# kurhula/pyABC

Measured on AMD Instinct MI355X. Metric: accepted particles/sec/generation, higher is better.
Workload: dtype f32 (f16x3-limb MFMA, f32-grade)

## Files before the change

### include/abcgpu.h

```cpp
#ifndef ABCGPU_H
#define ABCGPU_H

#include <stddef.h>
#include <stdint.h>

#ifdef __cplusplus
extern "C" {
#endif

#define ABC_OK 0
#define ABC_ERR_INVALID (-1)
#define ABC_ERR_HIP (-2)
#define ABC_ERR_WORKSPACE (-3)
#define ABC_ERR_NOT_ENOUGH_PARTICLES (-4)
#define ABC_ERR_UNSUPPORTED (-5)
#define ABC_ERR_COMM (-6)

#define ABC_MAX_D 2048

#define ABC_PREC_F64 0
#define ABC_PREC_F32 1
#define ABC_PREC_X3 2

#define ABC_PRIOR_FLAT (-1)
// ... 76 lines not shown

int abc_mask_gave_up(double* dist, const int32_t* attempts, int64_t B,
                     int max_attempts, double value, void* stream);

size_t abc_compact_workspace(int64_t B);
int abc_accept_compact(const double* d, int64_t B, double eps, int64_t* idx,
                       int64_t* count, void* ws, size_t ws_bytes,
                       void* stream);
typedef struct abc_candidate_spec {
  int d;
  int S;
  const double* X;
  const double* cdf;
  const int32_t* guide;
  int64_t N;
  const double* L;
  int per_particle_L;
  const int32_t* prior_kind;
  const double* prior_params;
  int max_attempts;
  const int32_t* src;
  const double* a;
  const double* sigma;
  const double* x0;
  const double* wf;
  double p;
  uint64_t seed;
  uint32_t generation;
  const void* anc_table;
  const double* support_box;
} abc_candidate_spec;
int abc_prior_support_box(const int32_t* prior_kind, const double* prior_params, int d,
                          double* box, void* stream);
int64_t abc_ancestor_table_bytes(int64_t N, int d);
int abc_ancestor_table(const double* X, const double* cdf, int64_t N, int d,
                       void* table, size_t table_bytes, void* stream);
size_t abc_candidates_workspace(int64_t B);
int abc_candidates_round(const abc_candidate_spec* spec, int64_t idx0,
                         int64_t B, double eps, const double* eps_dev,
                         double eps_scale, int filter, int64_t cap,
                         int64_t* idx, int64_t* count, double* rec_x,
                         void* ws, size_t ws_bytes, void* stream);
int abc_round_keep(const int64_t* counts, int nranks, int rank, int64_t need, int64_t* keep,
                   void* stream);
int abc_candidates_regen(const abc_candidate_spec* spec, int64_t idx0,
                         const int64_t* idx, int64_t n, const int64_t* n_dev,
                         double* theta, double* prior_logpdf, int64_t* ancestor,
                         double* x, double* dist, void* stream);

size_t abc_candidates_propose_workspace(void);
int abc_candidates_propose(const abc_candidate_spec* spec, int64_t idx0, int64_t B,
                           double* theta, double* prior_logpdf, int64_t* ancestor,
                           int32_t* attempts, void* ws, size_t ws_bytes, void* stream);

int abc_pnorm_accept(const double* x, int64_t B, int S, const double* x0,
                     const double* wf, double p, double eps, const int32_t* attempts,
                     int max_attempts, int64_t cap, int64_t* idx, int64_t* count,
                     void* ws, size_t ws_bytes, void* stream);

#define ABC_AGG_MAX_TERMS 16
int abc_aggregate_distance(const double* x, int64_t B, int S, const double* x0,
                           const double* wf, const double* p, const double* c, int K,
                           double* d, double* terms, void* stream);
int abc_aggregate_accept(const double* x, int64_t B, int S, const double* x0,
                         const double* wf, const double* p, const double* c, int K,
                         double eps, const int32_t* attempts, int max_attempts, int64_t cap,
                         int64_t* idx, int64_t* count, void* ws, size_t ws_bytes,
// ... 120 lines not shown
```

### pyabc_amd/_native.py

```python
import ctypes as C
import os
import threading

_HERE = os.path.dirname(os.path.abspath(__file__))
LIB_PATH = os.environ.get("ABCGPU_LIB", os.path.join(_HERE, "libabcgpu.so"))

P = C.c_void_p
I64 = C.c_int64
I32 = C.c_int
D = C.c_double
U64 = C.c_uint64
U32 = C.c_uint32
SZ = C.c_size_t

SIGNATURES = {
    "abc_last_error": (C.c_char_p, []),
    "abc_version": (I32, []),
    "abc_profile_begin": (I32, []),
    "abc_profile_end": (I32, [P, P]),
    "abc_profile_channel": (I32, [I32, P, P]),
    "abc_weighted_moments_workspace": (SZ, [I64, I32]),
    "abc_weighted_moments": (I32, [P, P, I64, I32, P, P, SZ, P]),
    "abc_scan_workspace": (SZ, [I64]),
    "abc_inclusive_scan_f64": (I32, [P, P, I64, P, SZ, P]),
    "abc_normalize_weights_workspace": (SZ, [I64]),
    "abc_normalize_weights": (I32, [P, I64, P, P, SZ, P]),
    "abc_mvn_packed_bytes": (SZ, [I64, I32, I32]),
    "abc_mvn_x3_layout": (I32, [I32, P, P]),
    "abc_mvn_x3_max_exponent": (I32, []),
    "abc_mvn_pack_population": (I32, [P, P, I64, I32, P, P, I32, D, P, I32, P, P,
                                      P]),
    "abc_mvn_fit": (I32, [P, I32, D, I32, P, P, P, P, P, P, P]),
    "abc_mvn_logpdf_workspace": (SZ, [I64, I64, I32, I32]),
    "abc_mvn_logpdf": (I32, [P, I64, I32, P, P, P, I64, P, P, I32, I32, D, D,
                             P, P, P, SZ, P]),
    "abc_mvn_logpdf_direct": (I32, [P, I64, P, P, I64, I32, P, I32, P, I32,
                                    D, D, P, P]),
    "abc_cdf_guide": (I32, [P, I64, P, P]),
    "abc_ancestor_table_bytes": (I64, [I64, I32]),
    "abc_ancestor_table": (I32, [P, P, I64, I32, P, SZ, P]),
    "abc_propose": (I32, [P, P, P, I64, I32, P, P, P, U64, U32, I64, I64, I32,
                          P, P, P, P, P]),
    "abc_prior_logpdf": (I32, [P, I64, I32, P, P, P, P]),
    "abc_prior_uniforms": (I32, [P, P, I64, I32, U64, U32, I64, P]),
    "abc_simulate_linear_gaussian": (I32, [P, I64, I32, I32, P, P, P, U64,
                                           U32, I64, P, P]),
    "abc_pnorm": (I32, [P, I64, I32, P, P, D, P, P]),
    "abc_mask_gave_up": (I32, [P, P, I64, I32, D, P]),
    "abc_compact_workspace": (SZ, [I64]),
    "abc_accept_compact": (I32, [P, I64, D, P, P, P, SZ, P]),
    "abc_candidates_workspace": (SZ, [I64]),
    "abc_prior_support_box": (I32, [P, P, I32, P, P]),
    "abc_round_keep": (I32, [P, I32, I32, I64, P, P]),
    "abc_candidates_round": (I32, [P, I64, I64, D, P, D, I32, I64, P, P, P, P, SZ, P]),
    "abc_candidates_regen": (I32, [P, I64, P, I64, P, P, P, P, P, P, P]),
    "abc_pnorm_accept": (I32, [P, I64, I32, P, P, D, D, P, I32, I64, P, P, P, SZ, P]),
    "abc_aggregate_distance": (I32, [P, I64, I32, P, P, P, P, I32, P, P, P]),
    "abc_aggregate_accept": (I32, [P, I64, I32, P, P, P, P, I32, D, P, I32, I64, P, P, P,
                                   SZ, P]),
    "abc_column_span": (I32, [P, I64, I32, P, P, SZ, P]),
    "abc_whitened_norm": (I32, [P, I64, I32, P, P, P, P]),
    "abc_whitened_accept": (I32, [P, I64, I32, P, P, D, P, I32, I64, P, P, P, SZ, P]),
    "abc_column_gram": (I32, [P, I64, I32, P, P, P, SZ, P]),
    "abc_column_quantile": (I32, [P, I64, I32, D, P, P, SZ, P]),
    "abc_candidates_propose_workspace": (SZ, []),
    "abc_candidates_propose": (I32, [P, I64, I64, P, P, P, P, P, SZ, P]),
    "abc_gather_rows": (I32, [P, P, I64, I32, P, P]),
    "abc_gather_rows_batch": (I32, [I32, P, P, P, P, P, I64, P]),
    "abc_importance_weights": (I32, [P, P, P, I64, D, P, P]),
    "abc_sort_pairs_workspace": (SZ, [I64]),
    "abc_sort_pairs_f64": (I32, [P, P, I64, P, P, P, SZ, P]),
    "abc_weighted_quantile_workspace": (SZ, [I64]),
# ... 121 lines not shown
```

### pyabc_amd/csrc/abc_candidate.h

```cpp
#pragma once
#include "abc_common.h"

#pragma clang fp contract(off)

namespace abc {

constexpr double LOG_SQRT_2PI = 0.91893853320467274178;
constexpr uint32_t SLOTS_PER_ATTEMPT = 65536;
constexpr uint32_t SLOT_ANCESTOR = 0;
constexpr uint32_t SLOT_PERTURB = 1;
constexpr uint32_t SLOT_PRIOR = 32;
constexpr uint32_t SLOT_SIM = 0x40000000u;

__device__ __forceinline__ void normals4(uint64_t g, uint32_t slot, uint32_t gen,
                                         uint64_t seed, double n[4], int need = 4,
                                         const float* tab = BM_TAB) {
  u32x4 r = philox(g, slot, gen, seed);
  box_muller(r.x, r.y, n[0], n[1], tab);
  if (need > 2) box_muller(r.z, r.w, n[2], n[3], tab);
}

__device__ __forceinline__ void perturb_words(int p, const u32x4& anc, u32x4& r, uint64_t g,
                                              uint32_t s0, uint32_t gen, uint64_t seed,
                                              uint32_t& wa, uint32_t& wb) {
// ... 288 lines not shown
      const uint64_t new_lo = f == 0 ? lo : lo + step * (uint64_t)f;
      lo = new_lo;
      hi = new_hi;
    }
    return hi;
  };
  const uint64_t kc = dkey(c);
  uint64_t lo_key;
  if (prior_in_support1(kind, p, -INFINITY)) lo_key = dkey(-INFINITY);
  else lo_key = turn(dkey(-INFINITY), kc, true);
  uint64_t hi_key;
  if (prior_in_support1(kind, p, INFINITY)) hi_key = dkey(INFINITY);
  else hi_key = turn(kc, dkey(INFINITY), false) - 1;
  if (lane == 0) { lo_hi[0] = dval(lo_key); lo_hi[1] = dval(hi_key); }
}

struct ProposalArgs {
  const double* X;
  const double* cdf;
  const int32_t* guide;
  int64_t N;
  const double* L;
  const int32_t* kind;
  const double* params;
  int d;
  int max_attempts;
  uint64_t seed;
  uint32_t gen;
  const double* rec = nullptr;
  const int32_t* bguide = nullptr;
  int rs = 0;
  int64_t G = 0;
  const double* xmax = nullptr;
};

constexpr int ANC_HDR = 256;
__host__ __device__ inline int anc_rs(int d) { return (d + 1 + 15) / 16 * 16; }
__host__ __device__ inline int64_t anc_bins(int64_t N) {
  const int64_t g = 4 * N;
  return g < (int64_t)0x7FFFFFF0 ? g : (int64_t)0x7FFFFFF0;
}
__device__ __forceinline__ int64_t anc_bin(double x, double inv_step, int64_t G) {
  const double b = x * inv_step;
  return b >= (double)G ? G : (int64_t)b;
}

constexpr int PROP_MVN = 0, PROP_LOCAL = 1, PROP_PRIOR = 2;
using PropModes = std::integer_sequence<int, PROP_MVN, PROP_LOCAL, PROP_PRIOR>;
inline int proposal_mode(const double* X, bool per_particle_L) {
  return X == nullptr ? PROP_PRIOR : (per_particle_L ? PROP_LOCAL : PROP_MVN);
}

using CandDims = std::integer_sequence<int, 1, 2, 3, 4, 5, 6, 8, 10, 12, 16>;

template <class F>
void dispatch_candidate(int d, int mode, F&& f) {
  auto with_d = [&](auto D) { dispatch_int(PropModes{}, mode, [&](auto MODE) { f(D, MODE); }); };
  if (!dispatch_int(CandDims{}, d, with_d)) with_d(std::integral_constant<int, 0>{});
}

struct SimDistArgs {
  const int32_t* src;
  const double* a;
  const double* sigma;
  const double* x0;
  const double* wf;
  double p;
  int S;
};

constexpr int SIM_SMAX = 256;
constexpr int LT_DMAX = 16;
struct BlockConsts {
  float bmt[BM_TAB_SIZE];
  double LT[LT_DMAX * LT_DMAX];
  double box[2 * 64];
  double2 as[SIM_SMAX];
  double2 wx[SIM_SMAX];
// ... 2 lines not shown
  double inv_step;
  int lazy;
};

template <int D, int MODE, bool BOX_FROM_SRC = false>
__device__ __forceinline__ void stage_block_consts(BlockConsts& C, const ProposalArgs& A,
                                                   const SimDistArgs* M,
                                                   const double* box_src) {
  const int t = threadIdx.x, nt = blockDim.x;
  const int d = D > 0 ? D : A.d;
  for (int k = t; k < BM_TAB_SIZE; k += nt) C.bmt[k] = BM_TAB[k];
  if (MODE == PROP_MVN && D > 0 && D <= LT_DMAX)
    for (int e = t; e < d * d; e += nt) C.LT[(e % d) * d + e / d] = A.L[e];
  if (BOX_FROM_SRC) {
    for (int k = t; k < 2 * d; k += nt) C.box[k] = box_src[k];
  } else {
    for (int k = t >> 6; k < d; k += nt >> 6)
      support_bounds_wave(A.kind[k], A.params + 4 * k, C.box + 2 * k);
  }
  if (M)
    for (int k = t; k < M->S && k < SIM_SMAX; k += nt) {
      C.as[k] = make_double2(M->a[k], M->sigma[k]);
      C.wx[k] = make_double2(M->wf[k], M->x0[k]);
      C.src[k] = M->src[k];
    }
  if (t == 0) {
    const double total = (MODE != PROP_PRIOR) ? A.cdf[A.N - 1] : 0.0;
    C.total = total;
    C.inv_step = (MODE != PROP_PRIOR && A.rec) ? (double)A.G / total : 0.0;
  }
  __syncthreads();
}

template <int D, int MODE, bool TABLE = false>
__device__ __forceinline__ int propose_one(const ProposalArgs& A, const BlockConsts& C,
                                           uint64_t g, double* th, int64_t& j) {
  constexpr bool LT_LDS = MODE == PROP_MVN && D > 0 && D <= LT_DMAX;
  const int d = D > 0 ? D : A.d;
  j = -1;
  const double total = C.total;
  for (int att = 0; att < A.max_attempts; ++att) {
    const uint32_t s0 = (uint32_t)att * SLOTS_PER_ATTEMPT;
    int oz = 0;
    asm volatile("" : "+s"(oz));
    const double* LT = C.LT + oz;
    const double* box = C.box + oz;
    if (MODE == PROP_PRIOR) {
#pragma unroll
      for (int k = 0; k < (D > 0 ? D : d); ++k)
        th[k] = prior_draw1(A.kind[k], A.params + 4 * k, g,
                            s0 + SLOT_PRIOR + 512u * k, A.gen, A.seed);
    } else {
      const u32x4 ra = philox(g, s0 + SLOT_ANCESTOR, A.gen, A.seed);
      u32x4 r = ra;
      const double target = uniform53(ra.x, ra.y) * total;
      AncestorBracket br;
      if (TABLE) {
        const int64_t kt = anc_bin(target, C.inv_step, A.G);
        br = {A.bguide[kt], A.bguide[kt + 1]};
      } else {
        br = ancestor_bracket(A.guide, A.N, total, target);
      }
#pragma unroll
      for (int k = 0; k < (D > 0 ? D : d); ++k) th[k] = 0.0;
      const double* Lj = A.L;
      if (MODE == PROP_LOCAL) {
        j = TABLE ? table_finish(A.rec, A.rs, d, A.N, target, br)
                  : ancestor_finish(A.cdf, A.N, target, br);
        Lj = A.L + j * d * d;
      }
      auto pair = [&](int q) {
        uint32_t wa, wb;
        perturb_words(q >> 1, ra, r, g, s0, A.gen, A.seed, wa, wb);
        double n0, n1;
        box_muller(wa, wb, n0, n1, C.bmt);
        const bool two = q + 1 < d;
#pragma unroll
        for (int k = 0; k < (D > 0 ? D : d); ++k) {
          if (k >= q) {
            const double l0 = LT_LDS ? LT[q * d + k] : Lj[k * d + q];
            th[k] = fma(l0, n0, th[k]);
          }
          if (two && k >= q + 1) {
            const double l1 = LT_LDS ? LT[(q + 1) * d + k] : Lj[k * d + q + 1];
            th[k] = fma(l1, n1, th[k]);
          }
        }
      };
#pragma unroll 1
      for (int q = 0; q < d; q += 2) pair(q);
      if (MODE != PROP_LOCAL)
        j = TABLE ? table_finish(A.rec, A.rs, d, A.N, target, br)
                  : ancestor_finish(A.cdf, A.N, target, br);
      const double* Xj = TABLE ? A.rec + j * A.rs : A.X + j * d;
#pragma unroll
      for (int k = 0; k < (D > 0 ? D : d); ++k) th[k] = Xj[k] + th[k];
    }
    bool ok = true;
#pragma unroll
    for (int k = 0; k < (D > 0 ? D : d); ++k)
      ok = ok & (box[2 * k] <= th[k]) & (th[k] <= box[2 * k + 1]);
    if (ok) return att + 1;
  }
  return A.max_attempts + 1;
}

constexpr int LAZY_KT = 4;

template <int D, int MODE>
__device__ __forceinline__ bool lazy_filter_ok(const BlockConsts& C, const ProposalArgs& A,
                                               const SimDistArgs& M) {
  if constexpr (MODE != PROP_MVN || D <= LAZY_KT || D > LT_DMAX) {
    return false;
  } else {
    if (A.xmax == nullptr || M.S <= 4) return false;
    bool ok = true;
    for (int k = 0; k < 4; ++k) ok = ok && C.src[k] >= 0 && C.src[k] < LAZY_KT;
    const double xm = *A.xmax;
    for (int k = LAZY_KT; k < D; ++k) {
      double ls = 0.0;
      for (int q = 0; q <= k; ++q) ls += fabs(C.LT[q * D + k]);
      const double b = (xm + 7.6 * ls) * 1.000001 + 1e-300;
      ok = ok && (C.box[2 * k] <= -b) && (b <= C.box[2 * k + 1]);
    }
    return ok;
  }
}

__device__ __forceinline__ double pterm(double v, double p) {
#pragma clang fp contract(off)
  return (p == 1.0) ? v : (p == 2.0 ? v * v : pow(v, p));
}
template <int PK = 0>
__device__ __forceinline__ double pnorm_acc(double s, double v, double p) {
#pragma clang fp contract(off)
  if constexpr (PK == 2) return s + v * v;
  return isinf(p) ? fmax(s, v) : s + pterm(v, p);
}
template <int PK = 0>
__device__ __forceinline__ double pnorm_finish(double s, double p) {
#pragma clang fp contract(off)
  if constexpr (PK == 2) return sqrt(s);
  return isinf(p) ? s : ((p == 1.0) ? s : (p == 2.0 ? sqrt(s) : pow(s, 1.0 / p)));
}
__device__ __forceinline__ double pnorm_row(const double* xr, int S, const double* x0,
                                            const double* wf, double p) {
#pragma clang fp contract(off)
  double s = 0.0;
// ... 77 lines not shown
    double n2[2];
    box_muller((q & 2) ? r.z : r.x, (q & 2) ? r.w : r.y, n2[0], n2[1], C.bmt);
#pragma unroll
    for (int t = 0; t < 2; ++t) {
      const int k = q + t;
      if (k < q1) {
        const double2 as = C.as[k], wx = C.wx[k];
        const int sk = __builtin_amdgcn_readfirstlane(C.src[k]);
        const double xv = lg_stat(as.x, as.y, th[sk], n2[t]);
        if (x) x[k - xoff] = xv;
        s = pnorm_acc<PK>(s, fabs(wx.x * (xv - wx.y)), M.p);
      }
    }
  }
  return s;
}

template <int D, int PK = 0>
__device__ __forceinline__ double sim_pnorm(const SimDistArgs& M, const BlockConsts& C,
                                            const double* th, uint64_t g, uint32_t gen,
                                            uint64_t seed, int q0, int q1, double s, double* x,
                                            int xoff = 0) {
  if constexpr (D > 0) {
    return sim_pnorm_regs<D, PK>(M, C, *reinterpret_cast<const double(*)[D]>(th), g, gen, seed,
                                 q0, q1, s, x, xoff);
  } else {
    return sim_pnorm_range<PK>(M, C, th, 1, g, gen, seed, q0, q1, s, x, xoff);
  }
}

template <int D, int PK, int CG>
__device__ __forceinline__ void lazy_head_group(const ProposalArgs& A, const SimDistArgs& M,
                                                const BlockConsts& C, const uint64_t (&g)[CG],
                                                double eps, bool (&keep)[CG]) {
  constexpr int KT = LAZY_KT;
  static_assert(D > KT, "lazy_head_group: D > LAZY_KT");
  int oz = 0;
  asm volatile("" : "+s"(oz));
  const double* LT = C.LT + oz;
  const double* box = C.box + oz;
  double target[CG];
  int32_t glo[CG], ghi[CG];
  uint32_t az[CG], aw[CG];
#pragma unroll
  for (int c = 0; c < CG; ++c) {
    const u32x4 r = philox(g[c], SLOT_ANCESTOR, A.gen, A.seed);
    target[c] = uniform53(r.x, r.y) * C.total;
    az[c] = r.z;
    aw[c] = r.w;
    const int64_t kt = anc_bin(target[c], C.inv_step, A.G);
    glo[c] = A.bguide[kt];
    ghi[c] = A.bguide[kt + 1];
  }
  double th[CG][KT];
#pragma unroll
  for (int c = 0; c < CG; ++c) {
#pragma unroll
    for (int k = 0; k < KT; ++k) th[c][k] = 0.0;
    const u32x4 r = philox(g[c], SLOT_PERTURB, A.gen, A.seed);
#pragma unroll
    for (int q = 0; q < KT; q += 2) {
      double n0, n1;
      box_muller(q == 0 ? az[c] : r.x, q == 0 ? aw[c] : r.y, n0, n1, C.bmt);
#pragma unroll
      for (int k = 0; k < KT; ++k) {
        if (k >= q) th[c][k] = fma(LT[q * D + k], n0, th[c][k]);
        if (k >= q + 1) th[c][k] = fma(LT[(q + 1) * D + k], n1, th[c][k]);
      }
    }
  }
  const double* xh[CG];
#pragma unroll
  for (int c = 0; c < CG; ++c) {
    const int64_t j = table_finish(A.rec, A.rs, D, A.N, target[c],
                                   AncestorBracket{(int64_t)glo[c], (int64_t)ghi[c]});
    xh[c] = A.rec + j * A.rs;
  }
  double xv4[CG][KT];
#pragma unroll
  for (int c = 0; c < CG; ++c)
#pragma unroll
    for (int k = 0; k < KT; ++k) xv4[c][k] = xh[c][k];
  double e[CG][4];
#pragma unroll
  for (int c = 0; c < CG; ++c) {
    const u32x4 r = philox(g[c], SLOT_SIM, A.gen, A.seed);
    box_muller(r.x, r.y, e[c][0], e[c][1], C.bmt);
    box_muller(r.z, r.w, e[c][2], e[c][3], C.bmt);
  }
#pragma unroll
  for (int c = 0; c < CG; ++c) {
    bool ok = true;
#pragma unroll
    for (int k = 0; k < KT; ++k) {
      th[c][k] = xv4[c][k] + th[c][k];
      ok = ok & (box[2 * k] <= th[c][k]) & (th[c][k] <= box[2 * k + 1]);
    }
    double s = 0.0;
#pragma unroll
    for (int k = 0; k < 4; ++k) {
      const double2 as = C.as[k], wx = C.wx[k];
      const int sk = __builtin_amdgcn_readfirstlane(C.src[k]);
      const double xv = lg_stat(as.x, as.y, th[c][sk], e[c][k]);
      s = pnorm_acc<PK>(s, fabs(wx.x * (xv - wx.y)), M.p);
    }
    keep[c] = !ok || !(pnorm_finish<PK>(s, M.p) > eps);
  }
}

}
```

### pyabc_amd/csrc/abc_fused.hip

```cpp
#include "abc_candidate.h"
#include "abc_aggregate.h"
#include "abc_accept_words.h"

namespace abc {
namespace {

constexpr int FR_T = 256;
constexpr int FR_CPT = 8;
constexpr int FR_TILE = FR_T * FR_CPT;
constexpr int FR_WORDS = FR_TILE / 64;
constexpr int FR_CG = 2;

struct RoundArgs {
  ProposalArgs P;
  SimDistArgs M;
  const double* box;
  const double* eps_dev;
  double eps_scale;
};

template <int D, int MODE, int PK>
__device__ __forceinline__ double evaluate_full(const RoundArgs& A, const BlockConsts& C,
                                                uint64_t g,
                                                double* th, int64_t& j, int& att, double* x) {
  att = propose_one<D, MODE, true>(A.P, C, g, th, j);
  const double s = sim_pnorm<D, PK>(A.M, C, th, g, A.P.gen, A.P.seed, 0, A.M.S, 0.0, x);
  const double dist = pnorm_finish<PK>(s, A.M.p);
  return att <= A.P.max_attempts ? dist : NAN;
}

constexpr int XCH = 16;
template <int D, int MODE, int PK>
__device__ __forceinline__ double evaluate_staged(const RoundArgs& A, const BlockConsts& C,
                                                  uint64_t g, bool valid, double* th,
                                                  int64_t& j, int& att, double* out,
                                                  int nvalid, double (*stage)[XCH + 1]) {
  const int t = threadIdx.x;
  const int S = A.M.S;
  att = valid ? propose_one<D, MODE, true>(A.P, C, g, th, j) : A.P.max_attempts + 1;
  double s = 0.0;
  for (int k0 = 0; k0 < S; k0 += XCH) {
    const int k1 = k0 + XCH < S ? k0 + XCH : S;
    if (valid) s = sim_pnorm<D, PK>(A.M, C, th, g, A.P.gen, A.P.seed, k0, k1, s, stage[t], k0);
    __syncthreads();
    const int w = k1 - k0;
    for (int e = t; e < FR_T * w; e += FR_T) {
      const int r = e / w, c = e - r * w;
      if (r < nvalid) out[(int64_t)r * S + k0 + c] = stage[r][c];
    }
    __syncthreads();
  }
  const double dist = pnorm_finish<PK>(s, A.M.p);
  return att <= A.P.max_attempts ? dist : NAN;
}

__device__ __forceinline__ void flush_accept_words(const uint32_t* tbits, int nwords,
                                                   int64_t tile0, int64_t B, uint64_t* bits) {
  const int lane = threadIdx.x & 63, wave = threadIdx.x >> 6;
  if (wave == 0 && lane < nwords) {
    const uint64_t w = (uint64_t)tbits[2 * lane] | ((uint64_t)tbits[2 * lane + 1] << 32);
    const int64_t word = tile0 / 64 + lane;
    if (word * 64 < B) bits[word] = w;
  }
}

struct TileLds {
  uint32_t* tbits;
  uint16_t* queue;
  int& qn;
};
template <int D, int MODE, bool FILTER, int PK>
__device__ __forceinline__ void tile_body(const RoundArgs& A, const BlockConsts& C, double eps,
                                          int64_t idx0, int64_t B, int64_t tile0, int cpt,
                                          uint64_t* __restrict__ bits,
                                          double* __restrict__ rec_x, TileLds T) {
  constexpr int DM = D > 0 ? D : 64;
  const int tid = threadIdx.x;
  const int tn = cpt * FR_T;
  if (tid < tn / 32) T.tbits[tid] = 0u;
  if (tid == 0) T.qn = 0;
  __syncthreads();
  double th[DM];
  int64_t j;
  int att;
  if (FILTER) {
    bool lazy_done = false;
    if constexpr (MODE == PROP_MVN && D > LAZY_KT && D <= LT_DMAX) {
      if (C.lazy) {
#pragma unroll 1
        for (int it = 0; it < cpt; it += FR_CG) {
          uint64_t gs[FR_CG];
          bool keep[FR_CG];
#pragma unroll
          for (int c = 0; c < FR_CG; ++c) gs[c] = (uint64_t)(idx0 + tile0 + (it + c) * FR_T + tid);
          lazy_head_group<D, PK, FR_CG>(A.P, A.M, C, gs, eps, keep);
#pragma unroll
          for (int c = 0; c < FR_CG; ++c) {
            const int loc = (it + c) * FR_T + tid;
            if (keep[c] && tile0 + loc < B) {
              const int pos = atomicAdd(&T.qn, 1);
              T.queue[pos] = (uint16_t)loc;
            }
          }
        }
        lazy_done = true;
      }
    }
#pragma unroll 1
    for (int it = 0; it < (lazy_done ? 0 : cpt); ++it) {
      const int loc = it * FR_T + tid;
      const int64_t b = tile0 + loc;
      if (b < B) {
        const uint64_t g = (uint64_t)(idx0 + b);
        att = propose_one<D, MODE, true>(A.P, C, g, th, j);
        const double s = sim_pnorm<D, PK>(A.M, C, th, g, A.P.gen, A.P.seed, 0, 4, 0.0, nullptr);
        if (att <= A.P.max_attempts && !(pnorm_finish<PK>(s, A.M.p) > eps)) {
          const int pos = atomicAdd(&T.qn, 1);
          T.queue[pos] = (uint16_t)loc;
        }
      }
    }
    __syncthreads();
  }
  const int n = FILTER ? T.qn : tn;
#pragma unroll 1
  for (int i = tid; i < n; i += FR_T) {
    const int loc = FILTER ? (int)T.queue[i] : i;
    const int64_t b = tile0 + loc;
    if (b < B) {
      double* xr = rec_x ? rec_x + b * A.M.S : nullptr;
      const double dist = evaluate_full<D, MODE, PK>(A, C, (uint64_t)(idx0 + b), th, j, att,
                                                  xr);
      if (dist <= eps) atomicOr(&T.tbits[loc >> 5], 1u << (loc & 31));
    }
  }
  __syncthreads();
  flush_accept_words(T.tbits, tn / 64, tile0, B, bits);
}

constexpr int FR_CPT_TAIL = 2;
constexpr int FR_TILE_TAIL = FR_T * FR_CPT_TAIL;

struct TilePlan {
  int64_t nbig, ntiles;
  unsigned int grid;
};
__host__ __device__ inline void tile_span(int64_t t, int64_t nbig, int64_t& tile0, int& cpt) {
  if (t < nbig) { tile0 = t * FR_TILE; cpt = FR_CPT; }
  else { tile0 = nbig * FR_TILE + (t - nbig) * FR_TILE_TAIL; cpt = FR_CPT_TAIL; }
}

template <int D, int MODE, bool FILTER, int PK>
__device__ __forceinline__ void round_body(RoundArgs A, int64_t idx0, int64_t B,
                                           double eps_host, uint64_t* __restrict__ bits,
                                           unsigned int* __restrict__ ticket,
                                           int64_t nbig, int64_t ntiles,
                                           double* __restrict__ rec_x) {
  const double eps = A.eps_dev ? (*A.eps_dev) * A.eps_scale : eps_host;
  __shared__ BlockConsts C;
  __shared__ uint32_t tbits[FR_TILE / 32];
  __shared__ uint16_t queue[FR_TILE];
  __shared__ int qn;
  __shared__ int64_t s_tile;
  const TileLds T{tbits, queue, qn};
  stage_block_consts<D, MODE, true>(C, A.P, &A.M, A.box);
  if (FILTER) {
    if (threadIdx.x == 0) C.lazy = lazy_filter_ok<D, MODE>(C, A.P, A.M) ? 1 : 0;
  }
  const unsigned int limit = (unsigned int)(ntiles + gridDim.x - 1);
#pragma unroll 1
  for (;;) {
    if (threadIdx.x == 0) s_tile = (int64_t)atomicInc(ticket, limit);
    __syncthreads();
    const int64_t t = s_tile;
    if (t >= ntiles) break;
    int64_t tile0;
    int cpt;
    tile_span(t, nbig, tile0, cpt);
    tile_body<D, MODE, FILTER, PK>(A, C, eps, idx0, B, tile0, cpt, bits, rec_x, T);
    __syncthreads();
  }
}

template <int D, int MODE, int PK>
__device__ __forceinline__ void round_plain_body(RoundArgs A, int64_t idx0, int64_t B,
                                                 double eps_host, uint64_t* __restrict__ bits,
                                                 unsigned int* __restrict__ ticket,
                                                 int64_t nbig, int64_t ntiles,
                                                 double* __restrict__ rec_x) {
  const double eps = A.eps_dev ? (*A.eps_dev) * A.eps_scale : eps_host;
  constexpr int DM = D > 0 ? D : 64;
  __shared__ BlockConsts C;
  __shared__ uint32_t tbits[FR_TILE / 32];
  __shared__ int64_t s_tile;
  stage_block_consts<D, MODE, true>(C, A.P, &A.M, A.box);
  const int tid = threadIdx.x, lane = tid & 63, wave = tid >> 6;
  const unsigned int limit = (unsigned int)(ntiles + gridDim.x - 1);
// ... 383 lines not shown
  unsigned long long a = 0ull;
  for (int64_t e = (int64_t)blockIdx.x * 256 + threadIdx.x; e < n; e += (int64_t)gridDim.x * 256) {
    const unsigned long long b = (unsigned long long)__double_as_longlong(fabs(X[e]));
    a = b > a ? b : a;
  }
#pragma unroll
  for (int o = 32; o > 0; o >>= 1) {
    const unsigned long long b = __shfl_xor(a, o, 64);
    a = b > a ? b : a;
  }
  if ((threadIdx.x & 63) == 0) wm[threadIdx.x >> 6] = a;
  __syncthreads();
  if (threadIdx.x == 0) {
    unsigned long long m = 0ull;
    for (int w = 0; w < 4; ++w) m = wm[w] > m ? wm[w] : m;
    atomicMax(xmax_bits, m);
  }
}

__global__ __launch_bounds__(256) void anc_guide_kernel(const double* __restrict__ cdf,
                                                        int64_t N, int64_t G,
                                                        int32_t* __restrict__ guide) {
  const int64_t k = (int64_t)blockIdx.x * 256 + threadIdx.x;
  if (k > G + 1) return;
  const double inv_step = (double)G / cdf[N - 1];
  int64_t lo = 0, hi = N;
  while (lo < hi) {
    const int64_t mid = (lo + hi) >> 1;
    if (anc_bin(cdf[mid], inv_step, G) >= k) hi = mid; else lo = mid + 1;
  }
  guide[k] = (int32_t)lo;
}

struct AncTable { const double* rec; const int32_t* guide; int rs; int64_t G; const double* xmax; };
inline AncTable anc_table_view(const void* t, int64_t N, int d) {
  AncTable v;
  v.xmax = static_cast<const double*>(t);
  v.rs = anc_rs(d);
  v.G = anc_bins(N);
  v.rec = reinterpret_cast<const double*>(static_cast<const char*>(t) + ANC_HDR);
  v.guide = reinterpret_cast<const int32_t*>(v.rec + N * v.rs);
  return v;
}

RoundArgs round_args(const abc_candidate_spec* s, const double* box) {
  RoundArgs A;
  A.box = box;
  A.eps_dev = nullptr;
  A.eps_scale = 1.0;
  A.P = ProposalArgs{s->X, s->cdf, s->guide, s->N, s->L, s->prior_kind,
                     s->prior_params, s->d, s->max_attempts, s->seed, s->generation};
  if (s->X && s->anc_table) {
    const AncTable v = anc_table_view(s->anc_table, s->N, s->d);
    A.P.rec = v.rec;
    A.P.bguide = v.guide;
    A.P.rs = v.rs;
    A.P.G = v.G;
    A.P.xmax = v.xmax;
  }
  A.M = SimDistArgs{s->src, s->a, s->sigma, s->x0, s->wf, s->p, s->S};
  return A;
}

int check_spec(const abc_candidate_spec* s) {
  ABC_CHECK_ARG(s != nullptr, "candidates: null spec");
  ABC_CHECK_ARG(s->d >= 1 && s->d <= 64 && s->S >= 1, "candidates: bad d/S");
  if (s->S > SIM_SMAX)
    return set_error(ABC_ERR_UNSUPPORTED, "candidates: S > %d (use the staged kernels)",
                     SIM_SMAX);
  ABC_CHECK_ARG(s->max_attempts >= 1 && s->max_attempts < (1 << 15),
                "candidates: bad max_attempts");
  ABC_CHECK_ARG(s->prior_kind && s->prior_params && s->src && s->a && s->sigma && s->x0 &&
                s->wf, "candidates: null pointer");
  ABC_CHECK_ARG(s->X == nullptr || (s->cdf && s->L && s->N >= 1),
                "candidates: population needs cdf, L, N");
  ABC_CHECK_ARG(s->p >= 1.0, "candidates: p < 1");
  ABC_CHECK_ARG(s->X == nullptr || s->anc_table, "candidates: population needs anc_table");
  return ABC_OK;
}

template <class F>
void dispatch_spec(const abc_candidate_spec* spec, F&& f) {
  dispatch_candidate(spec->d, proposal_mode(spec->X, spec->per_particle_L != 0), f);
}

}
}

using namespace abc;

struct RoundWs {
  unsigned int* ticket; int64_t* rtot; double* box; uint64_t* bits;
  void carve(Carver& c, int64_t B) {
    ticket = c.take<unsigned int>(64);
    rtot = c.take<int64_t>(RG_MAX);
    box = c.take<double>(128);
    bits = c.take<uint64_t>((size_t)ceil_div(B > 0 ? B : 1, FR_TILE) * FR_WORDS);
  }
};

extern "C" size_t abc_candidates_workspace(int64_t B) { return measure<RoundWs>(B); }

bool abc::accept_words_carve(void* ws, size_t ws_bytes, int64_t B, AcceptWords& w) {
  Carver cv(ws, ws_bytes);
  RoundWs r;
  r.carve(cv, B);
  w.bits = r.bits;
  w.rtot = r.rtot;
  return cv.ok;
}
int abc::accept_words_compact(const AcceptWords& w, int64_t B, int64_t cap, int64_t* idx,
                              int64_t* count, hipStream_t s) {
  return compact_accept_bits(w.bits, w.rtot, B, cap, idx, count, s);
}

extern "C" int64_t abc_ancestor_table_bytes(int64_t N, int d) {
  if (N < 1 || d < 1) return 0;
  return ANC_HDR + N * anc_rs(d) * (int64_t)sizeof(double) +
         (anc_bins(N) + 2) * (int64_t)sizeof(int32_t);
}

extern "C" int abc_ancestor_table(const double* X, const double* cdf, int64_t N, int d,
                                  void* table, size_t table_bytes, void* stream) {
  ABC_CHECK_ARG(N >= 1 && N < (1ll << 31) && d >= 1 && d <= 64,
                "ancestor_table: bad N/d");
  ABC_CHECK_ARG(X && cdf && table, "ancestor_table: null pointer");
  ABC_CHECK_ARG(((uintptr_t)table & 127) == 0, "ancestor_table: table not 128-B aligned");
  if ((int64_t)table_bytes < abc_ancestor_table_bytes(N, d))
    return set_error(ABC_ERR_WORKSPACE, "ancestor_table: buffer too small");
  const AncTable v = anc_table_view(table, N, d);
  hipStream_t s = as_stream(stream);
  ABC_HIP(hipMemsetAsync(table, 0, ANC_HDR, s));
  hipLaunchKernelGGL(anc_records_kernel, dim3((unsigned)ceil_div(N * v.rs, 256)), dim3(256), 0,
                     s, X, cdf, N, d, v.rs, const_cast<double*>(v.rec));
  ABC_LAUNCHED();
  const int64_t nx = N * (int64_t)d;
  const int64_t xb = ceil_div(nx, 256) < XMAX_BLOCKS ? ceil_div(nx, 256) : XMAX_BLOCKS;
  hipLaunchKernelGGL(anc_xmax_kernel, dim3((unsigned)xb), dim3(256), 0, s, X, nx,
                     static_cast<unsigned long long*>(table));
  ABC_LAUNCHED();
  hipLaunchKernelGGL(anc_guide_kernel, dim3((unsigned)ceil_div(v.G + 2, 256)), dim3(256), 0, s,
                     cdf, N, v.G, const_cast<int32_t*>(v.guide));
  ABC_LAUNCHED();
  return ABC_OK;
}

extern "C" int abc_candidates_round(const abc_candidate_spec* spec, int64_t idx0,
                                    int64_t B, double eps, const double* eps_dev,
                                    double eps_scale, int filter, int64_t cap,
                                    int64_t* idx, int64_t* count, double* rec_x,
                                    void* ws, size_t ws_bytes, void* stream) {
  const int rc = check_spec(spec);
  if (rc != ABC_OK) return rc;
  ABC_CHECK_ARG(B >= 0 && cap >= 0 && count, "candidates_round: bad B/cap/count");
  ABC_CHECK_ARG(B < (1ll << 40), "candidates_round: B too large");
  ABC_CHECK_ARG(cap == 0 || idx, "candidates_round: null idx");
  RoundWs w;
  ABC_CARVE(w, "candidates_round", B);
  hipStream_t s = as_stream(stream);
  if (B == 0) {
    ABC_HIP(hipMemsetAsync(count, 0, sizeof(int64_t), s));
    return ABC_OK;
  }
  const double p = spec->p;
  const int filt = (filter && rec_x == nullptr && spec->S > 4 &&
                    (p == 1.0 || p == 2.0 || p == INFINITY)) ? 1 : 0;
  const int64_t nt = ceil_div(B, FR_TILE);
  ABC_CHECK_ARG(nt < (1ll << 31), "candidates_round: too many tiles");
  const double* box = spec->support_box;
  if (!box) {
    hipLaunchKernelGGL(support_box_kernel, dim3((unsigned)spec->d), dim3(64), 0, s,
                       spec->prior_kind, spec->prior_params, spec->d, w.box);
    ABC_LAUNCHED();
    box = w.box;
  }
  RoundArgs A = round_args(spec, box);
// ... 153 lines not shown
```

### pyabc_amd/sampler/batched.py

```python
import logging
import math

import numpy as np

from .. import gpu
from .._native import PRIOR_KINDS
from ..distance.distance import SumStatMatrix
from ..population import ColumnarParticles, Particle, Population
from ..parameters import Parameter
from ..random_variables import host_prior_draw, host_prior_logpdf
from . import distributed as dd
from .base import Sampler

logger = logging.getLogger("Sampler")


class ColumnarSample:

    def __init__(self, columns, recorded, recorded_keys, record_rejected, ok,
                 accepted_flags=None, records=None):
        self._cols = columns
        self._records = records
        self._recorded = recorded
        self._recorded_keys = recorded_keys
# ... 361 lines not shown
        self.nr_evaluations_ = int(n_eval)
        self.last_stats = dict(rounds=0, evaluations=int(n_eval),
                               accepted=int(sample.n_accepted), per_candidate=True)
        return sample

    def _fused_round(self, spec, seed, gen, dev):
        if not self.fused or getattr(spec, "stochastic", None) is not None \
                or spec.distance is None or len(spec.param_names) > self.FUSED_MAX_DIM:
            return None
        if spec.transition is None and getattr(spec, "host_prior", None):
            return None
        sim = (spec.model.fused_simulator(dev)
               if hasattr(spec.model, "fused_simulator") else None)
        fp = (spec.distance.fused_pnorm(spec.t, spec.sum_stat_keys, dev)
              if hasattr(spec.distance, "fused_pnorm") else None)
        if sim is None or fp is None or len(spec.sum_stat_keys) > self.FUSED_MAX_STATS:
            return None
        prop = {}
        if spec.transition is not None:
            arrays = getattr(spec.transition, "proposal_arrays", None)
            if arrays is None:
                return None
            prop = arrays()
        src, a, sigma = sim
        wf, pval = fp
        fr = gpu.CandidateRound(len(spec.param_names), len(spec.sum_stat_keys),
                                spec.prior_kind, spec.prior_params, src, a,
                                sigma, spec.x0vec, wf, pval, seed, gen,
                                self.max_attempts, **prop)
        fr.src_host = getattr(spec.model, "src", None)
        return fr

    LAZY_KT = 4

    def _lazy_capable(self, spec, fr):
        s = fr.spec
        kinds = getattr(spec, "prior_kind_host", None)
        src = getattr(fr, "src_host", None)
        return (s.X is not None and not s.per_particle_L and s.d > self.LAZY_KT
                and s.S >= max(5, self.filter_min_stats) and s.p in (1.0, 2.0, math.inf)
                and kinds is not None
                and all(k in (PRIOR_KINDS["norm"], PRIOR_KINDS["laplace"])
                        for k in kinds)
                and src is not None and all(0 <= int(v) < self.LAZY_KT for v in src[:4]))

    FIRST_ROUND_SPARE = 4_000_000

    def _fused_size(self, need, ws, rate, measured, S, record):
        if self.batch_size is not None:
            return int(self.batch_size)
        r = rate if rate else 0.5
        if measured:
            mult = 1.06
        else:
            r *= self._acc_trend if rate else 1.0
            mult = 1.0 + min(0.1, self.FIRST_ROUND_SPARE * ws * max(r, 1e-12) / max(need, 1))
        b = need / max(r, 1e-12) * mult / ws + 4096
        cap = self.max_fused_batch_size
        if record:
            cap = min(cap, max(self.record_budget_bytes // (8 * S), 4096))
        return int(min(max(b, 4096), cap))

    def _limit_to_max_eval(self, B, max_eval, n_eval, ws):
        if not self.check_max_eval or not np.isfinite(max_eval):
            return B
        left = int(math.ceil(max_eval)) - int(n_eval)
        return int(max(1, min(B, left // ws)))

    def _ledger(self, n, rank, ws, S):
        return _RoundLedger(n, rank, ws, S, self.max_nr_recorded,
                            self.record_device_budget_bytes)

    def _sample_fused(self, n, fr, spec, max_eval, record, dev, rank, ws):
        torch = gpu.torch
        S = len(spec.sum_stat_keys)
        rec_x = []
        arena, arena_off = None, 0
        kept, kept_off, kept_segs = None, 0, []
        row_bytes = (8 * fr.d, 8, 8, 8 * S, 8)
        led = self._ledger(n, rank, ws, S)
        rate, measured = self._acc_rate, False
        tot_B = tot_cnt = 0
        filtered = reruns = 0
        while led.need > 0:
            if self.check_max_eval and led.n_eval >= max_eval:
                break
            need = led.need
            B = self._limit_to_max_eval(self._fused_size(need, ws, rate, measured, S, record),
                                        max_eval, led.n_eval, ws)
            kk = min(need, B)
            lo, _ = dd.rank_range(led.base, B, rank)
            rx = None
            if record and led.rec_left > 0:
                if arena is None or arena_off + B > arena.shape[0]:
                    arena = torch.empty((int(B * 1.25) + 4096, S), dtype=gpu.F64, device=dev)
                    arena_off = 0
                rx = arena[arena_off:arena_off + B]
            filt = (rate is not None and rate < self.filter_below and rx is None
                    and self._lazy_capable(spec, fr))
            filtered += int(filt)
            thr = getattr(spec, "eps_device", None) if led.rounds == 0 else None
            if thr is not None:
                idx, cnt = fr.run(lo, B, 0.0, cap=need, filter=filt, rec_x=rx,
                                  eps_dev=thr[0], eps_scale=thr[1])
            else:
                idx, cnt = fr.run(lo, B, spec.eps, cap=need, filter=filt, rec_x=rx)
            if ws == 1:
                n_keep = cnt
                self._reader.queue(cnt, idx[kk - 1:kk])
            else:
                gathered = dd.allgather_counts_device(cnt)
                n_keep = gpu.round_keep(gathered, need, rank)
                self._reader.queue(gathered)
            if kept is None or kept_off + kk > kept[1]:
                if kept is not None and kept_off:
                    kept_segs.append((kept[0], kept_off))
                views = self._kept_buffers(kk, fr.d, S, dev)
                kept = (views, views[0].shape[0], [v.data_ptr() for v in views])
                kept_off = 0
            fr.regen_into(lo, idx.data_ptr(), kk,
                          [a + kept_off * b for a, b in zip(kept[2], row_bytes)],
                          n_dev=n_keep)
            counts = self._reader.wait()
            pos = None
            if ws == 1:
                counts, pos = counts[:1], int(counts[1])
            if thr is not None:
                spec.eps_device = None
                if np.isnan(thr[2].get()[0]):
                    reruns += 1
                    continue
# ... 191 lines not shown
```

Measured before the change: 7.515 million.

## Add coarse head-bin ancestor lookup table and reuse filtered ancestor in full evaluation

Adds a coarser 'head bin' level to the ancestor table. Each bin records either a direct ancestor index, a small inline entry holding up to three rows' CDF cut points and the first four coordinates, or a fall-back to the guide search. The lazy head filter uses this to resolve most ancestors with one or two loads instead of a bracketed search. Filter survivors now carry their ancestor index through LDS so the full evaluation skips the second search. The sampler also turns the lazy filter on automatically below a small acceptance rate when the statistic count is small, which adds work when the filter rejects too few. The cost is an extra table-build kernel, a larger table and more LDS per block.

After: 7.296 million. 0.971x the previous value.

```diff
diff --git a/include/abcgpu.h b/include/abcgpu.h
--- a/include/abcgpu.h
+++ b/include/abcgpu.h
@@ -132,7 +132,9 @@
 } abc_candidate_spec;
 int abc_prior_support_box(const int32_t* prior_kind, const double* prior_params, int d,
                           double* box, void* stream);
+#define ABC_ANC_REGIONS 5
 int64_t abc_ancestor_table_bytes(int64_t N, int d);
+int abc_ancestor_table_layout(int64_t N, int d, int64_t* out);
 int abc_ancestor_table(const double* X, const double* cdf, int64_t N, int d,
                        void* table, size_t table_bytes, void* stream);
 size_t abc_candidates_workspace(int64_t B);
diff --git a/pyabc_amd/_native.py b/pyabc_amd/_native.py
--- a/pyabc_amd/_native.py
+++ b/pyabc_amd/_native.py
@@ -38,6 +38,7 @@
                                     D, D, P, P]),
     "abc_cdf_guide": (I32, [P, I64, P, P]),
     "abc_ancestor_table_bytes": (I64, [I64, I32]),
+    "abc_ancestor_table_layout": (I32, [I64, I32, P]),
     "abc_ancestor_table": (I32, [P, P, I64, I32, P, SZ, P]),
     "abc_propose": (I32, [P, P, P, I64, I32, P, P, P, U64, U32, I64, I64, I32,
                           P, P, P, P, P]),
diff --git a/pyabc_amd/csrc/abc_candidate.h b/pyabc_amd/csrc/abc_candidate.h
--- a/pyabc_amd/csrc/abc_candidate.h
+++ b/pyabc_amd/csrc/abc_candidate.h
@@ -344,6 +344,8 @@
   int rs = 0;
   int64_t G = 0;
   const double* xmax = nullptr;
+  const double* hbin = nullptr;
+  const int32_t* hguide = nullptr;
 };
 
 constexpr int ANC_HDR = 256;
@@ -356,6 +358,14 @@
   const double b = x * inv_step;
   return b >= (double)G ? G : (int64_t)b;
 }
+constexpr int ANC_HB_SHIFT = 3, ANC_HB_R = 1 << ANC_HB_SHIFT;
+constexpr int ANC_HB_ROWS = 3;
+constexpr int ANC_HB_DBL = 16;
+constexpr int32_t ANC_HB_ENTRY = -1, ANC_HB_GUIDE = -2;
+__host__ __device__ inline int64_t anc_head_bins(int64_t N) {
+  return (anc_bins(N) >> ANC_HB_SHIFT) + 1;
+}
+__host__ __device__ inline bool anc_has_head_bins(int d) { return d > 4 && d <= 16; }
 
 constexpr int PROP_MVN = 0, PROP_LOCAL = 1, PROP_PRIOR = 2;
 using PropModes = std::integer_sequence<int, PROP_MVN, PROP_LOCAL, PROP_PRIOR>;
@@ -424,9 +434,11 @@
   __syncthreads();
 }
 
-template <int D, int MODE, bool TABLE = false>
+template <int D, int MODE, bool TABLE = false, bool KNOWN = false>
 __device__ __forceinline__ int propose_one(const ProposalArgs& A, const BlockConsts& C,
-                                           uint64_t g, double* th, int64_t& j) {
+                                           uint64_t g, double* th, int64_t& j,
+                                           int64_t j0 = -1) {
+  static_assert(!KNOWN || TABLE, "propose_one: KNOWN needs the ancestor table");
   constexpr bool LT_LDS = MODE == PROP_MVN && D > 0 && D <= LT_DMAX;
   const int d = D > 0 ? D : A.d;
   j = -1;
@@ -446,10 +458,13 @@
       const u32x4 ra = philox(g, s0 + SLOT_ANCESTOR, A.gen, A.seed);
       u32x4 r = ra;
       const double target = uniform53(ra.x, ra.y) * total;
-      AncestorBracket br;
+      AncestorBracket br{0, 0};
+      const bool known = KNOWN && att == 0 && j0 >= 0;
       if (TABLE) {
-        const int64_t kt = anc_bin(target, C.inv_step, A.G);
-        br = {A.bguide[kt], A.bguide[kt + 1]};
+        if (!known) {
+          const int64_t kt = anc_bin(target, C.inv_step, A.G);
+          br = {A.bguide[kt], A.bguide[kt + 1]};
+        }
       } else {
         br = ancestor_bracket(A.guide, A.N, total, target);
       }
@@ -457,8 +472,8 @@
       for (int k = 0; k < (D > 0 ? D : d); ++k) th[k] = 0.0;
       const double* Lj = A.L;
       if (MODE == PROP_LOCAL) {
-        j = TABLE ? table_finish(A.rec, A.rs, d, A.N, target, br)
-                  : ancestor_finish(A.cdf, A.N, target, br);
+        j = known ? j0 : (TABLE ? table_finish(A.rec, A.rs, d, A.N, target, br)
+                                : ancestor_finish(A.cdf, A.N, target, br));
         Lj = A.L + j * d * d;
       }
       auto pair = [&](int q) {
@@ -482,8 +497,8 @@
 #pragma unroll 1
       for (int q = 0; q < d; q += 2) pair(q);
       if (MODE != PROP_LOCAL)
-        j = TABLE ? table_finish(A.rec, A.rs, d, A.N, target, br)
-                  : ancestor_finish(A.cdf, A.N, target, br);
+        j = known ? j0 : (TABLE ? table_finish(A.rec, A.rs, d, A.N, target, br)
+                                : ancestor_finish(A.cdf, A.N, target, br));
       const double* Xj = TABLE ? A.rec + j * A.rs : A.X + j * d;
 #pragma unroll
       for (int k = 0; k < (D > 0 ? D : d); ++k) th[k] = Xj[k] + th[k];
@@ -505,7 +520,7 @@
   if constexpr (MODE != PROP_MVN || D <= LAZY_KT || D > LT_DMAX) {
     return false;
   } else {
-    if (A.xmax == nullptr || M.S <= 4) return false;
+    if (A.xmax == nullptr || A.hguide == nullptr || M.S <= 4) return false;
     bool ok = true;
     for (int k = 0; k < 4; ++k) ok = ok && C.src[k] >= 0 && C.src[k] < LAZY_KT;
     const double xm = *A.xmax;
@@ -649,15 +664,18 @@
 template <int D, int PK, int CG>
 __device__ __forceinline__ void lazy_head_group(const ProposalArgs& A, const SimDistArgs& M,
                                                 const BlockConsts& C, const uint64_t (&g)[CG],
-                                                double eps, bool (&keep)[CG]) {
+                                                double eps, bool (&keep)[CG],
+                                                int64_t (&anc)[CG]) {
   constexpr int KT = LAZY_KT;
+  static_assert(KT == 4 && LT_DMAX == 16, "anc_has_head_bins, the entry layout");
   static_assert(D > KT, "lazy_head_group: D > LAZY_KT");
   int oz = 0;
   asm volatile("" : "+s"(oz));
   const double* LT = C.LT + oz;
   const double* box = C.box + oz;
   double target[CG];
-  int32_t glo[CG], ghi[CG];
+  int32_t kt[CG];
+  int32_t hg[CG];
   uint32_t az[CG], aw[CG];
 #pragma unroll
   for (int c = 0; c < CG; ++c) {
@@ -665,9 +683,8 @@
     target[c] = uniform53(r.x, r.y) * C.total;
     az[c] = r.z;
     aw[c] = r.w;
-    const int64_t kt = anc_bin(target[c], C.inv_step, A.G);
-    glo[c] = A.bguide[kt];
-    ghi[c] = A.bguide[kt + 1];
+    kt[c] = (int32_t)anc_bin(target[c], C.inv_step, A.G);
+    hg[c] = A.hguide[kt[c] >> ANC_HB_SHIFT];
   }
   double th[CG][KT];
 #pragma unroll
@@ -686,24 +703,54 @@
       }
     }
   }
-  const double* xh[CG];
+  int32_t glo[CG], ghi[CG];
+  double hc[CG][2], hx[CG][ANC_HB_ROWS][KT];
+  long long hi0[CG];
+  double xv4[CG][KT];
 #pragma unroll
   for (int c = 0; c < CG; ++c) {
-    const int64_t j = table_finish(A.rec, A.rs, D, A.N, target[c],
-                                   AncestorBracket{(int64_t)glo[c], (int64_t)ghi[c]});
-    xh[c] = A.rec + j * A.rs;
-  }
-  double xv4[CG][KT];
-#pragma unroll
-  for (int c = 0; c < CG; ++c)
-#pragma unroll
-    for (int k = 0; k < KT; ++k) xv4[c][k] = xh[c][k];
+    if (hg[c] >= 0) {
+      anc[c] = hg[c];
+      const double* xh = A.rec + anc[c] * A.rs;
+#pragma unroll
+      for (int k = 0; k < KT; ++k) xv4[c][k] = xh[k];
+    } else if (hg[c] == ANC_HB_GUIDE) {
+      glo[c] = A.bguide[kt[c]];
+      ghi[c] = A.bguide[kt[c] + 1];
+    } else {
+      const double* he = A.hbin + (int64_t)(kt[c] >> ANC_HB_SHIFT) * ANC_HB_DBL;
+      hi0[c] = __double_as_longlong(he[0]);
+      hc[c][0] = he[1];
+      hc[c][1] = he[2];
+#pragma unroll
+      for (int q = 0; q < ANC_HB_ROWS; ++q)
+#pragma unroll
+        for (int k = 0; k < KT; ++k) hx[c][q][k] = he[4 + q * KT + k];
+    }
+  }
   double e[CG][4];
 #pragma unroll
   for (int c = 0; c < CG; ++c) {
     const u32x4 r = philox(g[c], SLOT_SIM, A.gen, A.seed);
     box_muller(r.x, r.y, e[c][0], e[c][1], C.bmt);
     box_muller(r.z, r.w, e[c][2], e[c][3], C.bmt);
+  }
+#pragma unroll
+  for (int c = 0; c < CG; ++c) {
+    if (hg[c] == ANC_HB_GUIDE) {
+      anc[c] = table_finish(A.rec, A.rs, D, A.N, target[c],
+                            AncestorBracket{(int64_t)glo[c], (int64_t)ghi[c]});
+      const double* xh = A.rec + anc[c] * A.rs;
+#pragma unroll
+      for (int k = 0; k < KT; ++k) xv4[c][k] = xh[k];
+    } else if (hg[c] == ANC_HB_ENTRY) {
+      const int s0 = hc[c][0] > target[c] ? 0 : 1;
+      const int sel = s0 == 0 ? 0 : (hc[c][1] > target[c] ? 1 : 2);
+      anc[c] = (int64_t)hi0[c] + sel;
+#pragma unroll
+      for (int k = 0; k < KT; ++k)
+        xv4[c][k] = sel == 0 ? hx[c][0][k] : (sel == 1 ? hx[c][1][k] : hx[c][2][k]);
+    }
   }
 #pragma unroll
   for (int c = 0; c < CG; ++c) {
diff --git a/pyabc_amd/csrc/abc_fused.hip b/pyabc_amd/csrc/abc_fused.hip
--- a/pyabc_amd/csrc/abc_fused.hip
+++ b/pyabc_amd/csrc/abc_fused.hip
@@ -19,11 +19,12 @@
   double eps_scale;
 };
 
-template <int D, int MODE, int PK>
+template <int D, int MODE, int PK, bool KNOWN = false>
 __device__ __forceinline__ double evaluate_full(const RoundArgs& A, const BlockConsts& C,
                                                 uint64_t g,
-                                                double* th, int64_t& j, int& att, double* x) {
-  att = propose_one<D, MODE, true>(A.P, C, g, th, j);
+                                                double* th, int64_t& j, int& att, double* x,
+                                                int64_t j0 = -1) {
+  att = propose_one<D, MODE, true, KNOWN>(A.P, C, g, th, j, j0);
   const double s = sim_pnorm<D, PK>(A.M, C, th, g, A.P.gen, A.P.seed, 0, A.M.S, 0.0, x);
   const double dist = pnorm_finish<PK>(s, A.M.p);
   return att <= A.P.max_attempts ? dist : NAN;
@@ -67,6 +68,7 @@
 struct TileLds {
   uint32_t* tbits;
   uint16_t* queue;
+  int32_t* qanc;
   int& qn;
 };
 template <int D, int MODE, bool FILTER, int PK>
@@ -75,6 +77,7 @@
                                           uint64_t* __restrict__ bits,
                                           double* __restrict__ rec_x, TileLds T) {
   constexpr int DM = D > 0 ? D : 64;
+  constexpr bool KNOWN = FILTER && MODE != PROP_PRIOR;
   const int tid = threadIdx.x;
   const int tn = cpt * FR_T;
   if (tid < tn / 32) T.tbits[tid] = 0u;
@@ -91,15 +94,17 @@
         for (int it = 0; it < cpt; it += FR_CG) {
           uint64_t gs[FR_CG];
           bool keep[FR_CG];
+          int64_t ja[FR_CG];
 #pragma unroll
           for (int c = 0; c < FR_CG; ++c) gs[c] = (uint64_t)(idx0 + tile0 + (it + c) * FR_T + tid);
-          lazy_head_group<D, PK, FR_CG>(A.P, A.M, C, gs, eps, keep);
+          lazy_head_group<D, PK, FR_CG>(A.P, A.M, C, gs, eps, keep, ja);
 #pragma unroll
           for (int c = 0; c < FR_CG; ++c) {
             const int loc = (it + c) * FR_T + tid;
             if (keep[c] && tile0 + loc < B) {
               const int pos = atomicAdd(&T.qn, 1);
               T.queue[pos] = (uint16_t)loc;
+              T.qanc[pos] = (int32_t)ja[c];
             }
           }
         }
@@ -117,6 +122,7 @@
         if (att <= A.P.max_attempts && !(pnorm_finish<PK>(s, A.M.p) > eps)) {
           const int pos = atomicAdd(&T.qn, 1);
           T.queue[pos] = (uint16_t)loc;
+          if (KNOWN) T.qanc[pos] = att == 1 ? (int32_t)j : -1;
         }
       }
     }
@@ -129,8 +135,9 @@
     const int64_t b = tile0 + loc;
     if (b < B) {
       double* xr = rec_x ? rec_x + b * A.M.S : nullptr;
-      const double dist = evaluate_full<D, MODE, PK>(A, C, (uint64_t)(idx0 + b), th, j, att,
-                                                  xr);
+      const int64_t j0 = KNOWN ? (int64_t)T.qanc[i] : -1;
+      const double dist = evaluate_full<D, MODE, PK, KNOWN>(A, C, (uint64_t)(idx0 + b), th, j,
+                                                            att, xr, j0);
       if (dist <= eps) atomicOr(&T.tbits[loc >> 5], 1u << (loc & 31));
     }
   }
@@ -160,9 +167,10 @@
   __shared__ BlockConsts C;
   __shared__ uint32_t tbits[FR_TILE / 32];
   __shared__ uint16_t queue[FR_TILE];
+  __shared__ int32_t qanc[FR_TILE];
   __shared__ int qn;
   __shared__ int64_t s_tile;
-  const TileLds T{tbits, queue, qn};
+  const TileLds T{tbits, queue, qanc, qn};
   stage_block_consts<D, MODE, true>(C, A.P, &A.M, A.box);
   if (FILTER) {
     if (threadIdx.x == 0) C.lazy = lazy_filter_ok<D, MODE>(C, A.P, A.M) ? 1 : 0;
@@ -612,14 +620,82 @@
   guide[k] = (int32_t)lo;
 }
 
-struct AncTable { const double* rec; const int32_t* guide; int rs; int64_t G; const double* xmax; };
+struct HeadBin { int64_t lo; int nrow; int32_t code; };
+__device__ __forceinline__ HeadBin head_bin(const int32_t* __restrict__ guide, int64_t N,
+                                            int64_t G, int64_t kh) {
+  const int64_t k0 = kh << ANC_HB_SHIFT;
+  const int64_t k1 = k0 + ANC_HB_R < G + 1 ? k0 + ANC_HB_R : G + 1;
+  const int64_t lo = guide[k0], hi = guide[k1];
+  const int64_t last = hi < N ? hi : N - 1;
+  HeadBin h;
+  h.lo = lo;
+  h.nrow = (int)(last - lo + 1 < ANC_HB_ROWS + 1 ? last - lo + 1 : ANC_HB_ROWS + 1);
+  if (lo == hi || h.nrow <= 1) h.code = (int32_t)(lo < N ? lo : N - 1);
+  else h.code = h.nrow <= ANC_HB_ROWS ? ANC_HB_ENTRY : ANC_HB_GUIDE;
+  return h;
+}
+
+__global__ __launch_bounds__(256) void anc_head_bins_kernel(
+    const double* __restrict__ X, const double* __restrict__ cdf,
+    const int32_t* __restrict__ guide, int64_t N, int d, int64_t G, int64_t Gh,
+    double* __restrict__ hbin, int32_t* __restrict__ hguide) {
+  const int64_t e = (int64_t)blockIdx.x * 256 + threadIdx.x;
+  if (e >= Gh * ANC_HB_DBL) return;
+  const int64_t kh = e / ANC_HB_DBL;
+  const int slot = (int)(e - kh * ANC_HB_DBL);
+  const HeadBin h = head_bin(guide, N, G, kh);
+  if (slot == 0) hguide[kh] = h.code;
+  double v = 0.0;
+  if (h.code == ANC_HB_ENTRY) {
+    if (slot == 0) {
+      v = __longlong_as_double((long long)h.lo);
+    } else if (slot <= 2) {
+      v = slot - 1 < h.nrow - 1 ? cdf[h.lo + slot - 1] : INFINITY;
+    } else if (slot >= 4) {
+      const int c = (slot - 4) / LAZY_KT, k = (slot - 4) % LAZY_KT;
+      if (c < h.nrow && k < d) v = X[(h.lo + c) * d + k];
+    }
+  }
+  hbin[e] = v;
+}
+
+struct AncLayout {
+  int rs; int64_t G, Gh;
+  int64_t rec, guide, hbin, hguide;
+  int64_t bytes;
+};
+inline AncLayout anc_layout(int64_t N, int d) {
+  AncLayout a;
+  a.rs = anc_rs(d);
+  a.G = anc_bins(N);
+  a.Gh = anc_has_head_bins(d) ? anc_head_bins(N) : 0;
+  a.rec = ANC_HDR;
+  a.guide = a.rec + N * a.rs * (int64_t)sizeof(double);
+  a.bytes = a.guide + (a.G + 2) * (int64_t)sizeof(int32_t);
+  a.hbin = a.hguide = a.bytes;
+  if (a.Gh > 0) {
+    a.hbin = (a.bytes + 127) / 128 * 128;
+    a.hguide = a.hbin + a.Gh * ANC_HB_DBL * (int64_t)sizeof(double);
+    a.bytes = a.hguide + a.Gh * (int64_t)sizeof(int32_t);
+  }
+  return a;
+}
+struct AncTable {
+  const double* rec; const int32_t* guide; int rs; int64_t G; const double* xmax;
+  const double* hbin; const int32_t* hguide; int64_t Gh;
+};
 inline AncTable anc_table_view(const void* t, int64_t N, int d) {
+  const AncLayout a = anc_layout(N, d);
+  const char* base = static_cast<const char*>(t);
   AncTable v;
   v.xmax = static_cast<const double*>(t);
-  v.rs = anc_rs(d);
-  v.G = anc_bins(N);
-  v.rec = reinterpret_cast<const double*>(static_cast<const char*>(t) + ANC_HDR);
-  v.guide = reinterpret_cast<const int32_t*>(v.rec + N * v.rs);
+  v.rs = a.rs;
+  v.G = a.G;
+  v.Gh = a.Gh;
+  v.rec = reinterpret_cast<const double*>(base + a.rec);
+  v.guide = reinterpret_cast<const int32_t*>(base + a.guide);
+  v.hbin = a.Gh > 0 ? reinterpret_cast<const double*>(base + a.hbin) : nullptr;
+  v.hguide = a.Gh > 0 ? reinterpret_cast<const int32_t*>(base + a.hguide) : nullptr;
   return v;
 }
 
@@ -637,6 +713,8 @@
     A.P.rs = v.rs;
     A.P.G = v.G;
     A.P.xmax = v.xmax;
+    A.P.hbin = v.hbin;
+    A.P.hguide = v.hguide;
   }
   A.M = SimDistArgs{s->src, s->a, s->sigma, s->x0, s->wf, s->p, s->S};
   return A;
@@ -696,8 +774,23 @@
 
 extern "C" int64_t abc_ancestor_table_bytes(int64_t N, int d) {
   if (N < 1 || d < 1) return 0;
-  return ANC_HDR + N * anc_rs(d) * (int64_t)sizeof(double) +
-         (anc_bins(N) + 2) * (int64_t)sizeof(int32_t);
+  return anc_layout(N, d).bytes;
+}
+
+extern "C" int abc_ancestor_table_layout(int64_t N, int d, int64_t* out) {
+  ABC_CHECK_ARG(N >= 1 && d >= 1 && out, "ancestor_table_layout: bad N/d/out");
+  const AncLayout a = anc_layout(N, d);
+  const int64_t regions[ABC_ANC_REGIONS][2] = {
+      {0, ANC_HDR},
+      {a.rec, N * a.rs * (int64_t)sizeof(double)},
+      {a.guide, (a.G + 2) * (int64_t)sizeof(int32_t)},
+      {a.hbin, a.Gh * ANC_HB_DBL * (int64_t)sizeof(double)},
+      {a.hguide, a.Gh * (int64_t)sizeof(int32_t)}};
+  for (int r = 0; r < ABC_ANC_REGIONS; ++r) {
+    out[2 * r] = regions[r][0];
+    out[2 * r + 1] = regions[r][1];
+  }
+  return ABC_OK;
 }
 
 extern "C" int abc_ancestor_table(const double* X, const double* cdf, int64_t N, int d,
@@ -722,6 +815,12 @@
   hipLaunchKernelGGL(anc_guide_kernel, dim3((unsigned)ceil_div(v.G + 2, 256)), dim3(256), 0, s,
                      cdf, N, v.G, const_cast<int32_t*>(v.guide));
   ABC_LAUNCHED();
+  if (v.Gh > 0) {
+    hipLaunchKernelGGL(anc_head_bins_kernel, dim3((unsigned)ceil_div(v.Gh * ANC_HB_DBL, 256)),
+                       dim3(256), 0, s, X, cdf, v.guide, N, d, v.G, v.Gh,
+                       const_cast<double*>(v.hbin), const_cast<int32_t*>(v.hguide));
+    ABC_LAUNCHED();
+  }
   return ABC_OK;
 }
 
diff --git a/pyabc_amd/sampler/batched.py b/pyabc_amd/sampler/batched.py
--- a/pyabc_amd/sampler/batched.py
+++ b/pyabc_amd/sampler/batched.py
@@ -417,6 +417,13 @@
         return fr
 
     LAZY_KT = 4
+    LAZY_AUTO_BELOW = 1e-3
+    LAZY_AUTO_MAX_STATS = 16
+
+    def _filter_threshold(self, S):
+        if self.filter_below > 0:
+            return self.filter_below
+        return self.LAZY_AUTO_BELOW if S <= self.LAZY_AUTO_MAX_STATS else 0.0
 
     def _lazy_capable(self, spec, fr):
         s = fr.spec
@@ -481,7 +488,7 @@
                     arena = torch.empty((int(B * 1.25) + 4096, S), dtype=gpu.F64, device=dev)
                     arena_off = 0
                 rx = arena[arena_off:arena_off + B]
-            filt = (rate is not None and rate < self.filter_below and rx is None
+            filt = (rate is not None and rate < self._filter_threshold(S) and rx is None
                     and self._lazy_capable(spec, fr))
             filtered += int(filt)
             thr = getattr(spec, "eps_device", None) if led.rounds == 0 else None
```
